# petim0/fly_bProject

Measured on AMD Instinct MI355X. Metric: env-steps/sec (PPO rollout + update), 8192 envs per GPU, higher is better.
Workload: dtype f32 (optimizer step: fp16x2 operand split; rollout policy + critic: bf16x3 operand split; fp32 accumulate)

## Files before the change

### fly_bproject_amd/csrc/fs_common.inc

```
#ifndef FS_IN
#define FS_IN 73
#endif
#ifndef FS_RING
#define FS_RING 4
#endif
typedef short s16x4 __attribute__((ext_vector_type(4)));
constexpr int FS_PX = 96, FS_P1 = 256, FS_P2 = 128, FS_P4 = 32;
template <int PITCH>
__device__ __forceinline__ int fs_key(int r)
{
    if (PITCH % 128 == 0) return ((r & 3) << 2) | ((r >> 2) & 3);
    return (r >> 2) & 3;
}
template <int PITCH>
__device__ __forceinline__ int fs_off(int r, int c) { return r * PITCH + ((((c >> 3) ^ fs_key<PITCH>(r))) << 3) + (c & 7); }
template <int PITCH> constexpr int fs_plane() { return BM * PITCH; }

__device__ __forceinline__ void fs_mfma_v(f32x16& acc, const bf16x8& a, const bf16x8& b)
{
    asm volatile("v_mfma_f32_32x32x16_bf16 %0, %1, %2, %0" : "+v"(acc) : "v"(a), "v"(b));
}
__device__ __forceinline__ void fs_mfma_v0(f32x16& acc, const bf16x8& a, const bf16x8& b)
{
    asm volatile("v_mfma_f32_32x32x16_bf16 %0, %1, %2, 0" : "=&v"(acc) : "v"(a), "v"(b));
}
__device__ __forceinline__ void fs_mfma_vg(f32x16& acc, const bf16x8& a, const bf16x8& b)
{
    asm volatile("s_nop 3\n\tv_mfma_f32_32x32x16_bf16 %0, %1, %2, %0" : "+v"(acc) : "v"(a), "v"(b));
}
__device__ __forceinline__ void fs_mfma_vg0(f32x16& acc, const bf16x8& a, const bf16x8& b)
{
    asm volatile("s_nop 3\n\tv_mfma_f32_32x32x16_bf16 %0, %1, %2, 0" : "=&v"(acc) : "v"(a), "v"(b));
}
__device__ __forceinline__ void fs_mfma_settle(f32x16& acc) { asm volatile("s_nop 7\n\ts_nop 7\n\ts_nop 3" : "+v"(acc)); }
__device__ __forceinline__ void fs_mfma_settle(f32x16& a, f32x16& b) { asm volatile("s_nop 7\n\ts_nop 7\n\ts_nop 3" : "+v"(a), "+v"(b)); }

template <int K, int PITCH, bool SWAP, bool ZERO = true, int HEAD = B3_HEAD>
__device__ __forceinline__ void fs_gemm(const WeightHeadT<HEAD>& head, const u16* __restrict__ Wb, int tile0, const u16* act, int k0,
                                        f32x16& hi, f32x16& lo, int lane)
{
    constexpr int K16 = K / 16;
    constexpr int RING = K16 < FS_RING ? K16 : FS_RING;
    constexpr int ARING = K16 < B3_ARING ? K16 : B3_ARING;
    const int r = lane & 31;
    const int key = fs_key<PITCH>(r);
    const int sh = (k0 >> 3) + (lane >> 5);
    const u16* arow = act + r * PITCH;
    const u16* bp = Wb + (long)tile0 * K16 * 1536 + lane * 8;
    Frag3 b[RING], a[ARING];
    auto aload = [&](Frag3& f, int kb) {
        const u16* q = arow + (((sh + 2 * kb) ^ key) << 3);
#pragma unroll
        for (int p = 0; p < 3; ++p) f.p[p] = *reinterpret_cast<const float4*>(q + p * fs_plane<PITCH>());
    };
#pragma unroll
    for (int s = 0; s < RING; ++s) {
        if (s < ARING) aload(a[s], s);
#pragma unroll
        for (int p = 0; p < 3; ++p)
            b[s].p[p] = s < HEAD ? head.b[s].p[p] : *reinterpret_cast<const float4*>(bp + s * 1536 + p * 512);
    }
#pragma unroll
    for (int kb = 0; kb < K16; ++kb) {
        const int s = kb % RING, sa = kb % ARING;
        __builtin_amdgcn_sched_barrier(0);
        const bf16x8 w0 = as_bf16x8(b[s].p[0]), w1 = as_bf16x8(b[s].p[1]), w2 = as_bf16x8(b[s].p[2]);
        const bf16x8 x0 = as_bf16x8(a[sa].p[0]), x1 = as_bf16x8(a[sa].p[1]), x2 = as_bf16x8(a[sa].p[2]);
        if (ZERO && kb == 0) {
            if (!SWAP) { fs_mfma_v0(lo, w0, x2); fs_mfma_v0(hi, w0, x0); } else { fs_mfma_v0(lo, x2, w0); fs_mfma_v0(hi, x0, w0); }
        } else {
            if (!SWAP) { fs_mfma_v(lo, w0, x2); fs_mfma_v(hi, w0, x0); } else { fs_mfma_v(lo, x2, w0); fs_mfma_v(hi, x0, w0); }
        }
        if (!SWAP) { fs_mfma_v(lo, w2, x0); fs_mfma_v(lo, w1, x1); fs_mfma_v(lo, w0, x1); fs_mfma_v(lo, w1, x0); }
        else { fs_mfma_v(lo, x0, w2); fs_mfma_v(lo, x1, w1); fs_mfma_v(lo, x1, w0); fs_mfma_v(lo, x0, w1); }
        __builtin_amdgcn_sched_barrier(0);
        if (kb + RING < K16) {
#pragma unroll
            for (int p = 0; p < 3; ++p) b[s].p[p] = *reinterpret_cast<const float4*>(bp + (kb + RING) * 1536 + p * 512);
        }
        if (kb + ARING < K16) aload(a[sa], kb + ARING);
    }
    fs_mfma_settle(hi, lo);
    __builtin_amdgcn_sched_barrier(0);
}

template <int K, int PITCH, bool SWAP, bool ZERO, class E, int HOST_GAPS = 6 * (K / 16), int MODE = 0>
struct FsGemmHost {
    static constexpr bool SPLIT = MODE == 1;
    static constexpr int K16 = K / 16, GAPS = 6 * K16, HALF = K16 / 2;
    static constexpr int RING = K16 < FS_RING ? K16 : FS_RING;
    static constexpr int ARING = K16 < B3_ARING ? K16 : B3_ARING;
    static_assert(!SPLIT || K16 == 16, "the split order is written for K = 256");
    static_assert(HOST_GAPS <= GAPS && (MODE == 0 || HOST_GAPS <= 6 * HALF), "the guest must be done when the second half begins");
    static constexpr bool order_ok()
    {
        unsigned seen = 0;
        for (int i = 0; i < K16; ++i) {
            const int kb = kblock(i);
            if (kb < 0 || kb >= K16 || ((seen >> kb) & 1u)) return false;
            if (MODE == 1 && ((kb & 2) != 0) != (i >= HALF)) return false;
            seen |= 1u << kb;
        }
        return true;
    }
    Frag3 b[RING], a[ARING];
    const u16 *arow, *bp;
    int sh, key;
    f32x16 &hi, &lo;
    E& e;
    __device__ __forceinline__ FsGemmHost(f32x16& hi_, f32x16& lo_, E& e_) : hi(hi_), lo(lo_), e(e_) {}
    static constexpr int kblock(int i) { return !SPLIT ? i : (i < HALF ? 4 * (i >> 1) + (i & 1) : 4 * ((i - HALF) >> 1) + 2 + (i & 1)); }
    static_assert(order_ok(), "k-step order");
    __device__ __forceinline__ void aload(Frag3& f, int kb)
    {
        const u16* q = arow + (((sh + 2 * kb) ^ key) << 3);
#pragma unroll
        for (int p = 0; p < 3; ++p) f.p[p] = *reinterpret_cast<const float4*>(q + p * fs_plane<PITCH>());
    }
    __device__ __forceinline__ void bload(Frag3& f, int kb)
    {
#pragma unroll
        for (int p = 0; p < 3; ++p) f.p[p] = *reinterpret_cast<const float4*>(bp + kb * 1536 + p * 512);
    }
    template <int J>
    __device__ __forceinline__ void gap()
    {
        if constexpr (J < HOST_GAPS) {
            constexpr int T0 = J * E::TOTAL / HOST_GAPS, T1 = (J + 1) * E::TOTAL / HOST_GAPS;
            __builtin_amdgcn_sched_barrier(0);
            run<T0, T1>();
            __builtin_amdgcn_sched_barrier(0);
        }
    }
    template <int T, int TE>
    __device__ __forceinline__ void run()
    {
        if constexpr (T < TE) { e.q(T); run<T + 1, TE>(); }
    }
    template <int I>
    __device__ __forceinline__ void steps()
    {
        if constexpr (I < K16) {
            constexpr int s = I % RING, sa = I % ARING;
            if constexpr (MODE != 0 && I == HALF) {
                if (SPLIT) __syncthreads();
#pragma unroll
                for (int u = 0; u < ARING; ++u)
                    if (HALF + u < K16) aload(a[(HALF + u) % ARING], kblock(HALF + u));
            }
            __builtin_amdgcn_sched_barrier(0);
            const bf16x8 w0 = as_bf16x8(b[s].p[0]), w1 = as_bf16x8(b[s].p[1]), w2 = as_bf16x8(b[s].p[2]);
            const bf16x8 x0 = as_bf16x8(a[sa].p[0]), x1 = as_bf16x8(a[sa].p[1]), x2 = as_bf16x8(a[sa].p[2]);
            if constexpr (ZERO && I == 0) {
                if (!SWAP) { fs_mfma_v0(lo, w0, x2); gap<0>(); fs_mfma_v0(hi, w0, x0); } else { fs_mfma_v0(lo, x2, w0); gap<0>(); fs_mfma_v0(hi, x0, w0); }
            } else {
                if (!SWAP) { fs_mfma_v(lo, w0, x2); gap<6 * I>(); fs_mfma_v(hi, w0, x0); } else { fs_mfma_v(lo, x2, w0); gap<6 * I>(); fs_mfma_v(hi, x0, w0); }
            }
            gap<6 * I + 1>();
            if (!SWAP) {
                fs_mfma_v(lo, w2, x0); gap<6 * I + 2>(); fs_mfma_v(lo, w1, x1); gap<6 * I + 3>();
                fs_mfma_v(lo, w0, x1); gap<6 * I + 4>(); fs_mfma_v(lo, w1, x0);
            } else {
                fs_mfma_v(lo, x0, w2); gap<6 * I + 2>(); fs_mfma_v(lo, x1, w1); gap<6 * I + 3>();
                fs_mfma_v(lo, x1, w0); gap<6 * I + 4>(); fs_mfma_v(lo, x0, w1);
            }
            __builtin_amdgcn_sched_barrier(0);
            if constexpr (I + RING < K16) bload(b[s], kblock(I + RING));
            if constexpr (I + ARING < K16 && !(MODE != 0 && I < HALF && I + ARING >= HALF)) aload(a[sa], kblock(I + ARING));
            gap<6 * I + 5>();
            steps<I + 1>();
        }
    }
};
template <int K, int PITCH, bool SWAP, bool ZERO = true, int HEAD = B3_HEAD, int HOST_GAPS = 6 * (K / 16), int MODE = 0, class E>
__device__ __forceinline__ void fs_gemm_host(const WeightHeadT<HEAD>& head, const u16* __restrict__ Wb, int tile0, const u16* act, int k0,
                                             f32x16& hi, f32x16& lo, int lane, E& e)
{
    typedef FsGemmHost<K, PITCH, SWAP, ZERO, E, HOST_GAPS, MODE> G;
    G g(hi, lo, e);
    const int r = lane & 31;
    g.key = fs_key<PITCH>(r);
    g.sh = (k0 >> 3) + (lane >> 5);
    g.arow = act + r * PITCH;
    g.bp = Wb + (long)tile0 * G::K16 * 1536 + lane * 8;
    static_assert(MODE != 1 || HEAD <= 2, "a head is the first k-steps IN ORDER: 0, 1 are the split order's first two as well");
#pragma unroll
    for (int s = 0; s < G::RING; ++s) {
        if (s < G::ARING && (MODE == 0 || s < G::HALF)) g.aload(g.a[s], G::kblock(s));
        if (s < HEAD) {
#pragma unroll
            for (int p = 0; p < 3; ++p) g.b[s].p[p] = head.b[s].p[p];
        } else {
            g.bload(g.b[s], G::kblock(s));
        }
    }
    g.template steps<0>();
    fs_mfma_settle(hi, lo);
    __builtin_amdgcn_sched_barrier(0);
}

template <int T, int TE, class E>
__device__ __forceinline__ void fs_run_ops(E& e)
{
    if constexpr (T < TE) { e.q(T); fs_run_ops<T + 1, TE>(e); }
}
template <int J, int GAPS, class E>
__device__ __forceinline__ void fs_host_gap(E& e)
{
    __builtin_amdgcn_sched_barrier(0);
    fs_run_ops<J * E::TOTAL / GAPS, (J + 1) * E::TOTAL / GAPS>(e);
    __builtin_amdgcn_sched_barrier(0);
}
template <int J0, int GAPS, class E>
__device__ __forceinline__ void fs_dw_host(f32x16& acc, const bf16x8 (&z)[3], const bf16x8 (&a)[3], E& e)
{
    acc = __builtin_amdgcn_mfma_f32_32x32x16_bf16(z[0], a[2], acc, 0, 0, 0); fs_host_gap<J0 + 0, GAPS>(e);
    acc = __builtin_amdgcn_mfma_f32_32x32x16_bf16(z[2], a[0], acc, 0, 0, 0); fs_host_gap<J0 + 1, GAPS>(e);
    acc = __builtin_amdgcn_mfma_f32_32x32x16_bf16(z[1], a[1], acc, 0, 0, 0); fs_host_gap<J0 + 2, GAPS>(e);
    acc = __builtin_amdgcn_mfma_f32_32x32x16_bf16(z[0], a[1], acc, 0, 0, 0); fs_host_gap<J0 + 3, GAPS>(e);
    acc = __builtin_amdgcn_mfma_f32_32x32x16_bf16(z[1], a[0], acc, 0, 0, 0); fs_host_gap<J0 + 4, GAPS>(e);
    acc = __builtin_amdgcn_mfma_f32_32x32x16_bf16(z[0], a[0], acc, 0, 0, 0); fs_host_gap<J0 + 5, GAPS>(e);
}

template <int PITCH>
__device__ __forceinline__ void fs_store4(u16* plane0, int r, int c, const float4& y)
{
    unsigned a0, b0, c0, a1, b1, c1;
    split3x2(y.x, y.y, a0, b0, c0);
    split3x2(y.z, y.w, a1, b1, c1);
    u16* q = plane0 + fs_off<PITCH>(r, c);
    *reinterpret_cast<uint2*>(q) = make_uint2(a0, a1);
    *reinterpret_cast<uint2*>(q + fs_plane<PITCH>()) = make_uint2(b0, b1);
// ... 212 lines not shown
```

### fly_bproject_amd/csrc/mlp_fused_step.inc

```
#include "fs_common.inc"
constexpr int FS_OFF_X = 0;
constexpr int FS_X_HALVES = 3 * BM * FS_PX;
constexpr int FS_OFF_H1 = FS_OFF_X + 2 * FS_X_HALVES;
constexpr int FS_OFF_H2 = FS_OFF_H1 + 3 * BM * FS_P1;
constexpr int FS_OFF_H3 = FS_OFF_H2 + 3 * BM * FS_P2;
constexpr int FS_OFF_R = FS_OFF_H3 + 3 * BM * FS_P2;
constexpr int FS_OFF_Z4 = FS_OFF_R + 4 * BM * MLP_OUT * 2;
constexpr int FS_OFF_F32 = FS_OFF_R + 3 * BM * FS_P2;
constexpr int FS_TAIL_FLOATS = MLP_H1 + MLP_H2 + MLP_H3 + MLP_OUT + 2 * BM + 2 * MLP_OUT + 4;
constexpr int FS_XS_FLOATS = BM * MLP_IN;
constexpr int FS_LDS_BYTES = FS_OFF_F32 * 2 + FS_TAIL_FLOATS * 4;
static_assert(FS_OFF_Z4 + 3 * BM * FS_P4 <= FS_OFF_F32, "split-K partials and the dZ4 planes fit region R side by side");
static_assert(FS_XS_FLOATS * 4 <= 3 * BM * FS_P2 * 2, "the staging block fits H2's region");
static_assert(FS_LDS_BYTES <= 160 * 1024, "fits one CU");

template <int PITCH, bool DUMP>
__device__ __forceinline__ void fs_epilogue_elu(const f32x16& hi, const f32x16& lo, const float* bias, int col0, u16* plane0,
                                                int lane, float* __restrict__ dump_tile, int nvalid)
{
    const int r = lane & 31;
    float4 y[4];
#pragma unroll
    for (int g = 0; g < 4; ++g) {
        const int nb = col0 + acc_n(g, lane);
// ... 491 lines not shown
            f32x16 cs2;
            const bool more = tile + __builtin_amdgcn_readfirstlane(grid_v) < ntiles;
            FsXStoreSlices xc(xs, Xn, tl);
#pragma unroll
            for (int t = 0; t < 2; ++t) {
                const int ct = 2 * wave + t;
                bf16x8 z1f[2][3];
                {
                    f32x16 hi, lo;
                    if (t == 0) fs_gemm<MLP_H2, FS_P2, true>(wt2, PTB + MLP_OFF_PTB2, ct, Z2, 0, hi, lo, lane);
                    else fs_gemm<MLP_H2, FS_P2, true>(wt2b, PTB + MLP_OFF_PTB2, ct, Z2, 0, hi, lo, lane);
                    if (t == 0) { stamp<STAMP>(stamps, 12); if (!STAMP) fs_split(n); }
                    if (STAMP && t == 1) stamp<STAMP>(stamps, 16);
                    if (t == 0 && more) x_fetch(tile + __builtin_amdgcn_readfirstlane(grid_v), tl);
                    bf16x8 hf[2][3], zf[2][3];
#pragma unroll
                    for (int s = 0; s < 2; ++s) fs_trws<FS_P1>(hf[s], H1, tr1, ct, s);
                    fs_trws<FS_P2>(zf[0], Z2, tr2, 0, 0);
                    unsigned q[2][3][4];
                    const fs_u32x4 hw[2][3] = {{__builtin_bit_cast(fs_u32x4, hf[0][0]), __builtin_bit_cast(fs_u32x4, hf[0][1]),
                                                __builtin_bit_cast(fs_u32x4, hf[0][2])},
                                               {__builtin_bit_cast(fs_u32x4, hf[1][0]), __builtin_bit_cast(fs_u32x4, hf[1][1]),
                                                __builtin_bit_cast(fs_u32x4, hf[1][2])}};
                    FsDz1Ops<DUMP> ez(hi, lo, hw, q, DUMP ? dump.dz1 + row0 * MLP_H1 + ct * 1024 : nullptr, lane, nvalid);
#define FS_P8_STEP(C_)                                                                                                            \
                    {                                                                                                             \
                        constexpr int c = (C_), s = c >> 2, nt = c & 3;                                                           \
                        if (c + 1 < 8) fs_trws<FS_P2>(zf[(c + 1) & 1], Z2, tr2, (c + 1) & 3, (c + 1) >> 2);                        \
                        __builtin_amdgcn_sched_barrier(0);                                                                        \
                        fs_dw_host<6 * c, 48>(aW2[nt][t], zf[c & 1], hf[s], ez);                                                  \
                        if (STAMP && t == 0 && c == 3) stamp<STAMP>(stamps, 18);                                                  \
                        if (t == 0 && nt == wave) {                           \
                            if (s == 0) fs_colsum_step<true>(cs2, zf[c & 1]); else fs_colsum_step<false>(cs2, zf[c & 1]);         \
                        }                                                                                                         \
                        __builtin_amdgcn_sched_barrier(0);                                                                        \
                    }
                    FS_P8_STEP(0) FS_P8_STEP(1) FS_P8_STEP(2) FS_P8_STEP(3) FS_P8_STEP(4) FS_P8_STEP(5) FS_P8_STEP(6) FS_P8_STEP(7)
#undef FS_P8_STEP
                    if (STAMP && t == 0) stamp<STAMP>(stamps, 17);
                    bs1[t] += ez.zsum;
#pragma unroll
                    for (int s = 0; s < 2; ++s)
#pragma unroll
                        for (int p = 0; p < 3; ++p) {
                            const fs_u32x4 qq = {q[s][p][0], q[s][p][1], q[s][p][2], q[s][p][3]};
                            z1f[s][p] = __builtin_bit_cast(bf16x8, qq);
                        }
                }
                if (t == 0) {
                    bs2 += fs_colsum_done(cs2);
                    fs_dma_drain();
                    gemm_prefetch_b3<MLP_H2>(wt2b, PTB + MLP_OFF_PTB2, 2 * wave + 1, lane);
                }
                stamp<STAMP>(stamps, t == 0 ? 13 : 15);
                if (!STAMP) fs_split(n);
                {
                    bf16x8 af[2][2][3];
                    fs_trns<FS_PX>(af[0][0], Xc, trx, 0, 0);
                    fs_trns<FS_PX>(af[0][1], Xc, trx, 0, 1);
#pragma unroll
                    for (int kt = 0; kt < 3; ++kt) {
                        if (kt + 1 < 3) {
                            fs_trns<FS_PX>(af[(kt + 1) & 1][0], Xc, trx, kt + 1, 0);
                            fs_trns<FS_PX>(af[(kt + 1) & 1][1], Xc, trx, kt + 1, 1);
                        }
                        __builtin_amdgcn_sched_barrier(0);
                        fs_dw_fill3(aW1[t][kt], z1f[0], af[kt & 1][0], xc, 18 * t + 6 * kt);
                        fs_dw_fill3(aW1[t][kt], z1f[1], af[kt & 1][1], xc, 18 * t + 6 * kt + 3);
                        __builtin_amdgcn_sched_barrier(0);
                    }
                }
                if (t == 0) stamp<STAMP>(stamps, 14);
            }
        }
        stamp<STAMP>(stamps, 10);
        if (!STAMP) fs_split(n);
        __syncthreads();
        stamp<STAMP>(stamps, 11);
        if (!STAMP) fs_split(n);
    }
    if (STAMP) stamps = reinterpret_cast<unsigned long long*>(dump.out) + ((long)blockIdx.x * 64 + 63) * FS_STAMP_SLOTS;
    stamp<STAMP>(stamps, 0);
    if (!STAMP) fs_split(n);

    const int lane = tid & 63;
    const unsigned G = gridDim.x, wg = blockIdx.x;
    constexpr unsigned S1 = fs_pad256(FS_STRIDE1), S2 = fs_pad256(FS_STRIDE2), S3 = fs_pad256(FS_STRIDE3);
    const unsigned o1 = 0, o2 = G * S1, o3 = G * (S1 + S2), o4 = G * (S1 + S2 + S3);
#pragma unroll
    for (int t = 0; t < 2; ++t)
#pragma unroll
        for (int kt = 0; kt < 3; ++kt) fs_store_tile(ws, o1, G, wg, MLP_IN_PAD, 2 * wave + t, kt, aW1[t][kt], lane);
#pragma unroll
    for (int nt = 0; nt < 4; ++nt)
#pragma unroll
        for (int t = 0; t < 2; ++t) fs_store_tile(ws, o2, G, wg, MLP_H1, nt, 2 * wave + t, aW2[nt][t], lane);
#pragma unroll
    for (int a = 0; a < 2; ++a)
#pragma unroll
        for (int b = 0; b < 2; ++b) fs_store_tile(ws, o3, G, wg, MLP_H2, 2 * (wave >> 1) + a, 2 * (wave & 1) + b, aW3[a][b], lane);
    fs_store_tile(ws, o4, G, wg, MLP_H3, 0, wave, aW4, lane);
    if (lane < 32) {
        ws[fs_slab(o2, G, wg, MLP_H2 * MLP_H1 + 32 * wave + lane)] = bs2;
        ws[fs_slab(o3, G, wg, MLP_H3 * MLP_H2 + 32 * wave + lane)] = bs3;
        if (wave == 0) ws[fs_slab(o4, G, wg, MLP_OUT * MLP_H3 + lane)] = bs4;
    }
#pragma unroll
    for (int t = 0; t < 2; ++t) {
        const float v = bs1[t] + __shfl_xor(bs1[t], 32, 64);
        if (lane < 32) ws[fs_slab(o1, G, wg, MLP_H1 * MLP_IN_PAD + 32 * (2 * wave + t) + lane)] = v;
    }
    if (STAMP) {
        asm volatile("s_waitcnt vmcnt(0)" ::: "memory");
        stamp<STAMP>(stamps, 1);
        if (!STAMP) fs_split(n);
        if (threadIdx.x == 0) stamps[2] = realtime_cu();
    }
}

constexpr int FR_OFF_X = 0;
constexpr int FR_OFF_H1 = FR_OFF_X + FS_X_HALVES;
constexpr int FR_OFF_H2 = FR_OFF_H1 + 3 * BM * FS_P1;
constexpr int FR_OFF_H3 = FR_OFF_H2 + 3 * BM * FS_P2;
constexpr int FR_OFF_PART = FR_OFF_H3 + 3 * BM * FS_P2;
constexpr int FR_OFF_F32 = FR_OFF_PART + 4 * BM * MLP_OUT * 2;
constexpr int FR_TAIL_FLOATS = MLP_H1 + MLP_H2 + MLP_H3 + MLP_OUT + 3 * 32 + BM * MLP_NACT + 4;
constexpr int FR_LDS_BYTES = FR_OFF_F32 * 2 + FR_TAIL_FLOATS * 4;
static_assert(BM * MLP_IN * 4 <= 3 * BM * FS_P2 * 2, "the observation block fits H2's region");

struct FrLds {
    u16 *X, *H1, *H2, *H3;
    float *part, *bias1, *bias2, *bias3, *bias4, *sd, *lg, *varcur, *acts, *hld, *obs;
    __device__ __forceinline__ explicit FrLds(u16* lds)
        : X(lds + FR_OFF_X), H1(lds + FR_OFF_H1), H2(lds + FR_OFF_H2), H3(lds + FR_OFF_H3),
          part(reinterpret_cast<float*>(lds + FR_OFF_PART)), bias1(reinterpret_cast<float*>(lds + FR_OFF_F32)), bias2(bias1 + MLP_H1),
          bias3(bias2 + MLP_H2), bias4(bias3 + MLP_H3), sd(bias4 + MLP_OUT), lg(sd + 32), varcur(lg + 32), acts(varcur + 32),
          hld(acts + BM * MLP_NACT), obs(reinterpret_cast<float*>(lds + FR_OFF_H2)) {}
};

__device__ __forceinline__ void policy_tile_fs_setup(const FrLds& L, const float* __restrict__ P)
{
    const int tid = threadIdx.x;
    L.bias1[tid] = P[MLP_OFF_B1 + tid];
    if (tid < MLP_H2) L.bias2[tid] = P[MLP_OFF_B2 + tid];
    else L.bias3[tid - MLP_H2] = P[MLP_OFF_B3 + tid - MLP_H2];
    if (tid < MLP_OUT) L.bias4[tid] = P[MLP_OFF_B4 + tid];
}

__device__ __forceinline__ void policy_tile_fs_head(WeightHeadT<2>& w1, const u16* __restrict__ PB)
{
    const int wave = __builtin_amdgcn_readfirstlane(threadIdx.x >> 6);
    gemm_prefetch_b3<MLP_IN_PAD>(w1, PB + MLP_OFF_PB1, 2 * wave, threadIdx.x & 63);
}
template <bool STAMP = false, bool NORM = false>
__device__ __forceinline__ void policy_tile_fs(const FrLds& L, const long tile, const u16* __restrict__ PB, const float* __restrict__ x,
                                               const long n, float* __restrict__ v_out, const float* __restrict__ smp_eps,
                                               float* __restrict__ smp_act, float* __restrict__ smp_logp, const WeightHeadT<2>& w1,
                                               unsigned long long* stamps = nullptr, const float* norm_tab = nullptr)
{
    const int tid = threadIdx.x, wave = __builtin_amdgcn_readfirstlane(tid >> 6);
    int tl = tid;
    asm volatile("" : "+v"(tl));
    const int lane = tl & 63, r = lane & 31;
    const long row0 = tile * BM;
    const int nvalid = (int)(n - row0 < BM ? n - row0 : BM);
    const int lrow = tl >> 3, lq = tl & 7;
    const bool lin = lrow < nvalid;
    float eps_pre[4];
#pragma unroll
    for (int j = 0; j < 4; ++j)
        eps_pre[j] = (lin && 4 * lq + j < MLP_NACT) ? (smp_eps + row0 * MLP_NACT)[lrow * MLP_NACT + 4 * lq + j] : 0.0f;
    if (x != nullptr) {
        const long total = n * MLP_IN, base = tile * (BM * MLP_IN) + 584L * wave;
        for (int i = lane; i < 584; i += 64) L.obs[584 * wave + i] = base + i < total ? x[base + i] : 0.0f;
    }
    static_assert(BM * MLP_IN == 4 * 584, "eight rows per wave");
    if (tid < 32) {
        const float v = tid < MLP_NACT ? L.varcur[tid] : 1.0f;
        const float s = sqrtf(v);
        L.sd[tid] = s;
        float lg = tid < MLP_NACT ? logf(s) : 0.0f;
        L.lg[tid] = lg;
#pragma unroll
        for (int o = 1; o < 32; o <<= 1) lg += __shfl_xor(lg, o, 32);
        if (tid == 0) L.hld[0] = lg;
    }
    if (NORM) {
        float* row = L.obs + (tl >> 3) * FS_IN;
        const int c0 = 12 * (tl & 7);
#pragma unroll
        for (int j = 0; j < 12; ++j)
            if (c0 + j < FS_IN) row[c0 + j] = obs_norm_apply(row[c0 + j], norm_tab[c0 + j], norm_tab[FS_IN + c0 + j], norm_tab[2 * FS_IN]);
    }
    { FsXStoreSlices xc(L.obs, L.X, tl); xc.all(); }
    __syncthreads();
    stamp<STAMP>(stamps, 1);
    WeightHeadT<2> w4;
    {
        f32x16 hi, lo;
        WeightHeadT<2> w1b, w2a;
        fs_gemm<MLP_IN_PAD, FS_PX, false>(w1, PB + MLP_OFF_PB1, 2 * wave, L.X, 0, hi, lo, lane);
        gemm_prefetch_b3<MLP_IN_PAD>(w1b, PB + MLP_OFF_PB1, 2 * wave + 1, lane);
        fs_epilogue_elu<FS_P1, false>(hi, lo, L.bias1, 64 * wave, L.H1, lane, nullptr, nvalid);
        fs_gemm<MLP_IN_PAD, FS_PX, false>(w1b, PB + MLP_OFF_PB1, 2 * wave + 1, L.X, 0, hi, lo, lane);
        gemm_prefetch_b3<MLP_H2>(w2a, PB + MLP_OFF_PB2, wave, lane);
        fs_epilogue_elu<FS_P1, false>(hi, lo, L.bias1, 64 * wave + 32, L.H1, lane, nullptr, nvalid);
        __syncthreads();
        stamp<STAMP>(stamps, 2);
        WeightHeadT<2> w2b, w3;
        gemm_prefetch_b3<MLP_H2>(w2b, PB + MLP_OFF_PB2 + 3 * MLP_H2 * (MLP_H1 / 2), wave, lane);
        fs_gemm<MLP_H2, FS_P1, false>(w2a, PB + MLP_OFF_PB2, wave, L.H1, 0, hi, lo, lane);
        fs_gemm<MLP_H2, FS_P1, false, false>(w2b, PB + MLP_OFF_PB2 + 3 * MLP_H2 * (MLP_H1 / 2), wave, L.H1, MLP_H1 / 2, hi, lo, lane);
        gemm_prefetch_b3<MLP_H2>(w3, PB + MLP_OFF_PB3, wave, lane);
        fs_epilogue_elu<FS_P2, false>(hi, lo, L.bias2, 32 * wave, L.H2, lane, nullptr, nvalid);
        __syncthreads();
        stamp<STAMP>(stamps, 3);
        gemm_prefetch_b3<32>(w4, PB + MLP_OFF_PB4 + (long)(2 * wave) * 1536, 0, lane);
        fs_gemm<MLP_H2, FS_P2, false>(w3, PB + MLP_OFF_PB3, wave, L.H2, 0, hi, lo, lane);
        fs_epilogue_elu<FS_P2, false>(hi, lo, L.bias3, 32 * wave, L.H3, lane, nullptr, nvalid);
        __syncthreads();
        stamp<STAMP>(stamps, 4);
    }
    {
        f32x16 hi, lo;
        fs_gemm<32, FS_P2, false>(w4, PB + MLP_OFF_PB4 + (long)(2 * wave) * 1536, 0, L.H3, 32 * wave, hi, lo, lane);
        float* pw = L.part + wave * (BM * MLP_OUT);
#pragma unroll
        for (int g = 0; g < 4; ++g)
            *reinterpret_cast<float4*>(pw + r * MLP_OUT + 4 * ((acc_n(g, lane) >> 2) ^ ((r >> 1) & 7))) =
                make_float4(hi[4 * g] + lo[4 * g], hi[4 * g + 1] + lo[4 * g + 1], hi[4 * g + 2] + lo[4 * g + 2],
                            hi[4 * g + 3] + lo[4 * g + 3]);
    }
    __syncthreads();
    stamp<STAMP>(stamps, 5);
    {
        const int c0 = 4 * lq;
        const int cs = 4 * (lq ^ ((lrow >> 1) & 7));
        const float4 p0 = *reinterpret_cast<const float4*>(L.part + lrow * MLP_OUT + cs);
        const float4 p1 = *reinterpret_cast<const float4*>(L.part + BM * MLP_OUT + lrow * MLP_OUT + cs);
        const float4 p2 = *reinterpret_cast<const float4*>(L.part + 2 * BM * MLP_OUT + lrow * MLP_OUT + cs);
        const float4 p3 = *reinterpret_cast<const float4*>(L.part + 3 * BM * MLP_OUT + lrow * MLP_OUT + cs);
        const float4 b4 = *reinterpret_cast<const float4*>(L.bias4 + c0);
        const float4 s4 = *reinterpret_cast<const float4*>(L.sd + c0);
        const float hld = L.hld[0];
        const float zz[4] = {(((p0.x + p1.x) + p2.x) + p3.x) + b4.x, (((p0.y + p1.y) + p2.y) + p3.y) + b4.y,
                             (((p0.z + p1.z) + p2.z) + p3.z) + b4.z, (((p0.w + p1.w) + p2.w) + p3.w) + b4.w};
        const float sdv[4] = {s4.x, s4.y, s4.z, s4.w};
        float a[4], xsq[4], yv[4];
#pragma unroll
        for (int j = 0; j < 4; ++j) {
            const int col = c0 + j;
            const float y = (col < MLP_NACT) ? elu(zz[j]) : ((col == MLP_NACT) ? zz[j] : 0.0f);
            yv[j] = y;
            a[j] = 0.0f; xsq[j] = 0.0f;
            if (col < MLP_NACT && lin) {
                a[j] = y + sdv[j] * eps_pre[j];
                const float xj = (a[j] - y) / sdv[j];
                xsq[j] = xj * xj;
            }
        }
        const float M = fs_sum8((xsq[0] + xsq[1]) + (xsq[2] + xsq[3]));
        if (lin) {
            if (v_out && lq == MLP_NACT / 4) (v_out + row0)[lrow] = yv[MLP_NACT % 4];
#pragma unroll
            for (int j = 0; j < 4; ++j)
                if (c0 + j < MLP_NACT) {
                    const float ac = fminf(fmaxf(a[j], -1.0f), 1.0f);
                    (smp_act + row0 * MLP_NACT)[lrow * MLP_NACT + c0 + j] = ac;
                    L.acts[lrow * MLP_NACT + c0 + j] = ac;
                }
            if (lq == 0) (smp_logp + row0)[lrow] = gauss_logp(M, hld);
        }
    }
    __syncthreads();
}
```

### fly_bproject_amd/csrc/mlp_mfma.hip

```cpp
#include <hip/hip_runtime.h>
#include <stdint.h>
#include <type_traits>
#include <cstdio>
#include <cstdlib>
#include "flyhip.h"
#include "mlp_layout.h"
#include "obs_norm.h"
#include "domain_rand.h"
#include "launch.h"

namespace {

#include "loss_head.inc"
#include "mlp_gemm.inc"
#include "fs_stamp.inc"
#include "mlp_forward.inc"
#include "mlp_backward.inc"
#include "mlp_grad_w.inc"
#include "mlp_fused_step.inc"
#include "mlp_adam.inc"
#include "fly_body.inc"

constexpr int RS_LDS_FLOATS = FWD_LDS_FLOATS > ENVS_PER_BLOCK * FLY_NUM_OBS ? FWD_LDS_FLOATS : ENVS_PER_BLOCK * FLY_NUM_OBS;
constexpr int RS_B3_LDS_FLOATS = FWD_B3_LDS_FLOATS > ENVS_PER_BLOCK * FLY_NUM_OBS ? FWD_B3_LDS_FLOATS : ENVS_PER_BLOCK * FLY_NUM_OBS;
static_assert(ENVS_PER_BLOCK == BM && BLOCK == THREADS, "one forward tile = one env block");
constexpr int NORM_LDS_FLOATS = OBS_NORM_TABLE + 1;
static_assert(MLP_IN == OBS_NORM_COLS && OBS_NORM_TABLE <= THREADS, "one table entry per thread");

template <bool B3, bool NORM = false, bool DR = false>
__global__ __launch_bounds__(THREADS, B3 ? 1 : 2) void rollout_step_kernel(
    const FlyConfig* __restrict__ c, FlyBuffers b, const float* __restrict__ P, const void* __restrict__ PF,
    const float* __restrict__ x, long n, const float* __restrict__ eps, const float* __restrict__ var, int var_steps,
    float var_decay, float var_min, float* __restrict__ act, float* __restrict__ logp, float* __restrict__ v_out,
    const int* __restrict__ var_base)
{
    constexpr int ARENA = B3 ? RS_B3_LDS_FLOATS : RS_LDS_FLOATS;
    __shared__ __attribute__((aligned(16))) float lds[ARENA + (NORM ? NORM_LDS_FLOATS : 0)];
    float* const norm_tab = NORM ? lds + ARENA : nullptr;
    if (NORM) obs_norm_load(norm_tab, c);
    var_steps -= var_base ? *var_base : 0;
    constexpr int PH_ALL = PH_SCALE | PH_RESET | PH_INTEGRATE | PH_OBS | PH_PROGRESS | PH_REWARD;
    FlyRegs st;
    fly_load<PH_ALL, DR>(st, c, b, blockIdx.x);
    if (NORM) __syncthreads();
    if (B3)
        forward_body_b3<false, false, NORM>(lds, blockIdx.x, 1L << 40, P, static_cast<const u16*>(PF), x, n, nullptr, v_out, nullptr,
                                            nullptr, nullptr, nullptr, eps, var, act, logp, nullptr, var_steps, var_decay, var_min,
                                            nullptr, nullptr, false, norm_tab);
    else
        forward_body<false, false, NORM>(lds, blockIdx.x, 1L << 40, P, static_cast<const float*>(PF), x, n, nullptr, v_out, nullptr,
                                         nullptr, nullptr, nullptr, eps, var, act, logp, nullptr, var_steps, var_decay, var_min,
                                         norm_tab);
    __builtin_amdgcn_fence(__ATOMIC_RELEASE, "workgroup");
    __builtin_amdgcn_s_waitcnt(0);
    __syncthreads();
    fly_body<PH_ALL, DR>(c, act, b, lds, blockIdx.x, st);
}

__device__ __forceinline__ void store_pose(float* __restrict__ poses, int t, const FlyRegs& nx)
{
    const int sub = threadIdx.x;
    if (sub >= LANES_PER_ENV) return;
    float* p = poses + (long)t * FLY_POSE_FLOATS;
    if (sub < FLY_NUM_LEGS) {
#pragma unroll
        for (int i = 0; i < 3; ++i) p[7 + 3 * sub + i] = nx.jq[i];
    }
    if (sub == LANES_PER_ENV - 1) {
        p[0] = nx.r.px; p[1] = nx.r.py; p[2] = nx.r.pz; p[3] = nx.r.qx; p[4] = nx.r.qy; p[5] = nx.r.qz; p[6] = nx.r.qw;
    }
}

template <bool B3, int WPS, bool REC, bool NORM = false, bool DR = false>
__global__ __launch_bounds__(THREADS, WPS) void rollout_all_kernel(
    const FlyConfig* __restrict__ c, FlyBuffers b, const float* __restrict__ P, const void* __restrict__ PF,
    float* __restrict__ obs_ring, long n, const float* __restrict__ eps_all, const float* __restrict__ var, float var_decay,
    float var_min, float* __restrict__ act_all, float* __restrict__ logp_all, float* __restrict__ v_ring,
    float* __restrict__ reward_all, int T, const int* __restrict__ rows_applied, int64_t* __restrict__ reset_rows,
    int64_t* __restrict__ progress_rows, float* __restrict__ poses)
{
    constexpr int ARENA = B3 ? RS_B3_LDS_FLOATS : RS_LDS_FLOATS;
    __shared__ __attribute__((aligned(16))) float lds[ARENA + 32 + BM * MLP_NACT + (NORM ? NORM_LDS_FLOATS : 0)];
    float* const norm_tab = NORM ? lds + ARENA + 32 + BM * MLP_NACT : nullptr;
    if (NORM) obs_norm_load(norm_tab, c);
    constexpr int PH_ALL = PH_SCALE | PH_RESET | PH_INTEGRATE | PH_OBS | PH_PROGRESS | PH_REWARD;
    float* varcur = lds + ARENA;
    float* acts = B3 ? lds + ARENA + 32 : nullptr;
    if (threadIdx.x < MLP_NACT) varcur[threadIdx.x] = var[threadIdx.x];
    FlyRegs st;
    fly_load<PH_ALL, DR>(st, c, b, blockIdx.x);
    __syncthreads();
    const bool whole = (long)(blockIdx.x + 1) * BM <= n;
    for (int t = 0; t < T; ++t) {
        const float* x = obs_ring + (long)t * n * FLY_NUM_OBS;
        float* act = act_all + (long)t * n * MLP_NACT;
        b.obs = obs_ring + (long)(t + 1) * n * FLY_NUM_OBS;
        b.reward = reward_all + (long)t * n;
        if (reset_rows) { b.reset = reset_rows + (long)t * n; b.progress = progress_rows + (long)t * n; }
        const bool in_lds = B3 && whole;
        if (B3)
            forward_body_b3<false, false, NORM>(lds, blockIdx.x, 1L << 40, P, static_cast<const u16*>(PF), x, n, nullptr,
                                                v_ring + (long)t * n, nullptr, nullptr, nullptr, nullptr, eps_all + (long)t * n * MLP_NACT,
                                                varcur, act, logp_all + (long)t * n, nullptr, 0, var_decay, var_min,
                                                in_lds && t > 0 ? lds : nullptr, in_lds ? acts : nullptr, t > 0, norm_tab);
        else
            forward_body<false, false, NORM>(lds, blockIdx.x, 1L << 40, P, static_cast<const float*>(PF), x, n, nullptr,
                                             v_ring + (long)t * n, nullptr, nullptr, nullptr, nullptr, eps_all + (long)t * n * MLP_NACT,
                                             varcur, act, logp_all + (long)t * n, nullptr, 0, var_decay, var_min, norm_tab);
        if (!in_lds) {
            __builtin_amdgcn_fence(__ATOMIC_RELEASE, "workgroup");
            __builtin_amdgcn_s_waitcnt(0);
        }
        __syncthreads();
        FlyRegs nx;
        fly_body<PH_ALL, DR>(c, act, b, lds, blockIdx.x, st, &nx, in_lds ? acts : nullptr);
        if (REC && blockIdx.x == 0) store_pose(poses, t, nx);
        st = nx;
        if (threadIdx.x < MLP_NACT && var_decay > 0.0f) varcur[threadIdx.x] = fmaxf(var_min, varcur[threadIdx.x] - var_decay);
        if (!in_lds) asm volatile("s_waitcnt vmcnt(0)" ::: "memory");
        __syncthreads();
    }
}

template <bool STAMP, bool MULTI, bool REC, bool NORM = false, bool DR = false>
__global__ __launch_bounds__(THREADS, 1) void rollout_all_fs_kernel(
    const FlyConfig* __restrict__ c, FlyBuffers b, const float* __restrict__ P, const u16* __restrict__ PB,
    float* __restrict__ obs_ring, long n, const float* __restrict__ eps_all, const float* __restrict__ var, float var_decay,
    float var_min, float* __restrict__ act_all, float* __restrict__ logp_all, float* __restrict__ v_ring,
    float* __restrict__ reward_all, int T, int64_t* __restrict__ reset_rows, int64_t* __restrict__ progress_rows,
    void* __restrict__ aux)
{
    static_assert(!(STAMP && REC) && !(STAMP && NORM) && !(STAMP && DR), "the stamped diagnostic form neither records, normalises nor randomises");
    unsigned long long* const stamps = static_cast<unsigned long long*>(aux);
    float* const poses = static_cast<float*>(aux);
    extern __shared__ __attribute__((aligned(16))) u16 fr_lds[];
    const FrLds L(fr_lds);
    constexpr int PH_ALL = PH_SCALE | PH_RESET | PH_INTEGRATE | PH_OBS | PH_PROGRESS | PH_REWARD;
    policy_tile_fs_setup(L, P);
    float* const norm_tab = NORM ? reinterpret_cast<float*>(fr_lds) + FR_LDS_BYTES / 4 : nullptr;
    if (NORM) obs_norm_load(norm_tab, c);
    int64_t* const reset0 = b.reset;
    int64_t* const progress0 = b.progress;
    const long ntiles = n / BM;
    long tile = blockIdx.x;
    do {
        unsigned long long* st_tile = STAMP ? stamps + tile * (T + 1) * 8 : nullptr;
        if (threadIdx.x < 32) L.varcur[threadIdx.x] = threadIdx.x < MLP_NACT ? var[threadIdx.x] : 1.0f;
        b.reset = reset0; b.progress = progress0;
        FlyRegs st;
        fly_load<PH_ALL, DR>(st, c, b, (int)tile);
        WeightHeadT<2> w1;
        policy_tile_fs_head(w1, PB);
        __syncthreads();
        if (STAMP && threadIdx.x == 0) st_tile[6] = realtime_cu();
        for (int t = 0; t < T; ++t) {
            stamp<STAMP>(st_tile, 8 * t);
            float* act = act_all + (long)t * n * MLP_NACT;
            b.obs = obs_ring + (long)(t + 1) * n * FLY_NUM_OBS;
            b.reward = reward_all + (long)t * n;
            if (reset_rows) { b.reset = reset_rows + (long)t * n; b.progress = progress_rows + (long)t * n; }
            policy_tile_fs<STAMP, NORM>(L, tile, PB, t == 0 ? obs_ring : nullptr, n, v_ring + (long)t * n, eps_all + (long)t * n * MLP_NACT,
                                        act, logp_all + (long)t * n, w1, STAMP ? st_tile + 8 * t : nullptr, norm_tab);
            stamp<STAMP>(st_tile, 8 * t + 7);
            policy_tile_fs_head(w1, PB);
            FlyRegs nx;
            fly_body<PH_ALL, DR>(c, act, b, L.obs, (int)tile, st, &nx, L.acts);
            if (REC && tile == 0) store_pose(poses, t, nx);
            st = nx;
            if (threadIdx.x < MLP_NACT && var_decay > 0.0f) L.varcur[threadIdx.x] = fmaxf(var_min, L.varcur[threadIdx.x] - var_decay);
            __syncthreads();
        }
        stamp<STAMP>(st_tile, 8 * T);
        if (STAMP && threadIdx.x == 0) st_tile[8 * T + 1] = realtime_cu();
        tile += gridDim.x;
    } while (MULTI && tile < ntiles);
}

}

extern "C" hipError_t flyhip_launch_rollout_all(const FlyConfig* dcfg, const FlyBuffers* b, const float* P, const float* PF,
                                                float* obs_ring, int64_t n, const float* eps_all, const float* var,
                                                float var_decay, float var_min, float* act_all, float* logp_all, float* v_ring,
                                                float* reward_all, int T, const int* rows_applied, const uint16_t* PB,
                                                int64_t* reset_rows, int64_t* progress_rows, void* stream,
                                                unsigned long long* stamps, float* poses, int norm, int dr)
{
    const dim3 grid((unsigned)((n + BM - 1) / BM));
    const int cus = device_cus();
    const bool one_per_cu = (int)grid.x <= cus;
    const char* fs_env = getenv("FLY_ROLLOUT_FS");
    const bool fs_off = fs_env != nullptr && fs_env[0] == '0';
    if (stamps && (poses || norm || dr)) return hipErrorInvalidValue;
    const bool rec = poses != nullptr;
    if (PB && n % BM == 0 && !fs_off) {
        const dim3 grid_fs(one_per_cu ? grid.x : (unsigned)cus);
        static_assert(FR_LDS_BYTES % 4 == 0, "the table follows the image");
        auto fs = [&](void* aux, auto S, auto M, auto R, auto N, auto D) {
            return launch_kernel<rollout_all_fs_kernel<S.value, M.value, R.value, N.value, D.value>>(
                grid_fs, THREADS, FR_LDS_BYTES + (N.value ? NORM_LDS_FLOATS * 4 : 0), stream, dcfg, *b, P, PB, obs_ring, (long)n, eps_all,
                var, var_decay, var_min, act_all, logp_all, v_ring, reward_all, T, reset_rows, progress_rows, aux);
        };
        constexpr std::false_type no{};
        const bool multi = !one_per_cu;
        if (stamps) return with_bools([&](auto M) { return fs(stamps, std::true_type{}, M, no, no, no); }, multi);
        return with_bools([&](auto M, auto R, auto N, auto D) { return fs(poses, no, M, R, N, D); }, multi, rec, norm != 0, dr != 0);
    }
    if (stamps) return hipErrorInvalidValue;
    auto ra = [&](auto B3, auto WPS, const void* pf) {
        return with_bools([&](auto R, auto N, auto D) {
            return launch_kernel<rollout_all_kernel<B3.value, WPS.value, R.value, N.value, D.value>>(
                grid, THREADS, 0, stream, dcfg, *b, P, pf, obs_ring, (long)n, eps_all, var, var_decay, var_min, act_all, logp_all, v_ring,
                reward_all, T, rows_applied, reset_rows, progress_rows, poses);
        }, rec, norm != 0, dr != 0);
    };
    if (PB) return ra(std::true_type{}, int_c<1>{}, PB);
    return one_per_cu ? ra(std::false_type{}, int_c<1>{}, PF) : ra(std::false_type{}, int_c<2>{}, PF);
}

extern "C" hipError_t flyhip_launch_mlp_forward(const float* P, const float* PF, const float* x, int64_t n, float* mu_out,
                                                float* v_out, float* out_save, float* h1_save, float* h2_save,
                                                float* h3_save, const uint16_t* PB, void* stream)
{
    if (PB) {
        const long tiles = (n + BM - 1) / BM;
        const int grid = (int)tiles;
        hipLaunchKernelGGL(mlp_forward_b3_kernel, dim3(grid), dim3(THREADS), 0, (hipStream_t)stream, P, PB, x, (long)n, mu_out,
                           v_out, out_save, h1_save, h2_save, h3_save, (const float*)nullptr, (const float*)nullptr,
                           (float*)nullptr, (float*)nullptr, 0, 0.0f, 0.0f, (const int*)nullptr);
        return hipGetLastError();
    }
    const long tiles = (n + BM - 1) / BM;
    const int grid = (int)(tiles <= 4 * PERSIST_GRID ? tiles : PERSIST_GRID);
    hipLaunchKernelGGL(mlp_forward_kernel<false>, dim3(grid), dim3(THREADS), 0, (hipStream_t)stream, P, PF, x, (long)n,
                       mu_out, v_out, out_save, h1_save, h2_save, h3_save, (const float*)nullptr, (const float*)nullptr,
                       (float*)nullptr, (float*)nullptr, (unsigned long long*)nullptr, 0, 0.0f, 0.0f, (const int*)nullptr);
    return hipGetLastError();
}

extern "C" hipError_t flyhip_launch_mlp_forward_sample(const float* P, const float* PF, const float* x, int64_t n,
                                                       const float* eps, const float* var, int var_steps,
                                                       float var_decay, float var_min, float* act_out,
                                                       float* logp_out, float* mu_out, float* v_out, const uint16_t* PB,
                                                       const int* var_base, void* stream)
{
    if (PB) {
        const long tiles = (n + BM - 1) / BM;
        const int grid = (int)tiles;
        hipLaunchKernelGGL(mlp_forward_b3_kernel, dim3(grid), dim3(THREADS), 0, (hipStream_t)stream, P, PB, x, (long)n, mu_out,
                           v_out, (float*)nullptr, (float*)nullptr, (float*)nullptr, (float*)nullptr, eps, var, act_out,
                           logp_out, var_steps, var_decay, var_min, var_base);
        return hipGetLastError();
    }
    const long tiles = (n + BM - 1) / BM;
    const int grid = (int)(tiles <= 4 * PERSIST_GRID ? tiles : PERSIST_GRID);
    hipLaunchKernelGGL(mlp_forward_kernel<false>, dim3(grid), dim3(THREADS), 0, (hipStream_t)stream, P, PF, x, (long)n,
                       mu_out, v_out, (float*)nullptr, (float*)nullptr, (float*)nullptr, (float*)nullptr, eps,
                       var, act_out, logp_out, (unsigned long long*)nullptr, var_steps, var_decay, var_min, var_base);
    return hipGetLastError();
}

extern "C" int flyhip_debug_mlp_forward_stamped(const float* P, const float* PF, const float* x, int64_t n,
                                                float* out_save, float* h1_save, float* h2_save, float* h3_save,
                                                unsigned long long* stamps, void* stream, int grid_override)
{
    const long tiles = (n + BM - 1) / BM;
    const int grid = grid_override > 0 ? grid_override : (int)(tiles <= 4 * PERSIST_GRID ? tiles : PERSIST_GRID);
    hipLaunchKernelGGL(mlp_forward_kernel<true>, dim3(grid), dim3(THREADS), 0, (hipStream_t)stream, P, PF, x, (long)n,
                       (float*)nullptr, (float*)nullptr, out_save, h1_save, h2_save, h3_save, (const float*)nullptr,
                       (const float*)nullptr, (float*)nullptr, (float*)nullptr, stamps, 0, 0.0f, 0.0f, (const int*)nullptr);
    return (int)hipGetLastError();
}

extern "C" hipError_t flyhip_launch_mlp_backward_dx(const float* PT, const float* out_saved, const float* h1,
                                                    const float* h2, const float* h3, const float* action,
                                                    const float* old_logp, const float* adv, const float* target,
                                                    const float* var, int64_t n, float inv_batch, float clip,
                                                    float* dz4, float* dz3, float* dz2, float* dz1, float* loss_part,
                                                    const uint16_t* PTB, void* stream)
{
    if (PTB) {
        hipLaunchKernelGGL(mlp_backward_dx_b3_kernel, dim3((unsigned)((n + BM - 1) / BM)), dim3(THREADS), 0, (hipStream_t)stream,
                           PTB, out_saved, h1, h2, h3, action, old_logp, adv, target, var, (long)n, inv_batch, clip, dz4, dz3,
                           dz2, dz1, loss_part);
        return hipGetLastError();
    }
    const int grid = (int)((n + BM - 1) / BM);
    hipLaunchKernelGGL(mlp_backward_dx_kernel, dim3(grid), dim3(THREADS), 0, (hipStream_t)stream, PT, out_saved,
                       h1, h2, h3, action, old_logp, adv, target, var, (long)n, inv_batch, clip, dz4, dz3, dz2, dz1,
                       loss_part);
    return hipGetLastError();
}

static int kGradWgs[4] = {80, 100, 52, 24};
static int kGradWgsB3[4] = {72, 88, 64, 32};
static bool gw_env_read = false;
static void gw_read_env()
{
    if (gw_env_read) return;
    gw_env_read = true;
    const char* e = getenv("FLYHIP_GW_SPLIT");
    int v[4];
    if (e && sscanf(e, "%d,%d,%d,%d", &v[0], &v[1], &v[2], &v[3]) == 4 && v[0] > 0 && v[1] > 0 && v[2] > 0 && v[3] > 0 &&
        v[0] + v[1] + v[2] + v[3] <= 1024)
        for (int i = 0; i < 4; ++i) kGradWgs[i] = kGradWgsB3[i] = v[i];
}

static int g_fb_consumer_shift = 0;
extern "C" void flyhip_debug_set_fwd_bwd_consumer_shift(int shift) { g_fb_consumer_shift = shift; }

extern "C" hipError_t flyhip_launch_mlp_fwd_bwd(const float* P, const float* PF, const float* PT, const float* x, int64_t n,
                                                float* out_save, float* h1_save, float* h2_save, float* h3_save,
                                                const float* action, const float* old_logp, const float* adv,
                                                const float* target, const float* var, float inv_batch, float clip,
                                                float* dz4, float* dz3, float* dz2, float* dz1, float* loss_part,
                                                int* flags, int epoch, int* err, const uint16_t* PB, const uint16_t* PTB,
// ... 169 lines not shown
```

Before: 70.57 million.

## Keep layer-2 and output-head policy weights resident in AGPRs across rollout steps

Layer-2 and output-layer weight fragments are loaded once per kernel into accumulation registers (AGPRs) and reused on every timestep and tile. A new GEMM variant feeds MFMA directly from those registers instead of streaming weights from global memory through a prefetch ring. This removes repeated weight loads from the rollout loop. In exchange it holds a large block of AGPRs for the whole kernel, which can cut occupancy or cause spills.

Measured after the change: 70.91 million, median of 6. About the same (+0.5%).

```diff
diff --git a/fly_bproject_amd/csrc/fs_common.inc b/fly_bproject_amd/csrc/fs_common.inc
--- a/fly_bproject_amd/csrc/fs_common.inc
+++ b/fly_bproject_amd/csrc/fs_common.inc
@@ -78,6 +78,58 @@
 #pragma unroll
             for (int p = 0; p < 3; ++p) b[s].p[p] = *reinterpret_cast<const float4*>(bp + (kb + RING) * 1536 + p * 512);
         }
+        if (kb + ARING < K16) aload(a[sa], kb + ARING);
+    }
+    fs_mfma_settle(hi, lo);
+    __builtin_amdgcn_sched_barrier(0);
+}
+
+struct FragA { bf16x8 p[3]; };
+__device__ __forceinline__ void fs_hold(FragA& f)
+{
+#pragma unroll
+    for (int p = 0; p < 3; ++p) asm volatile("" : "+a"(f.p[p]));
+}
+__device__ __forceinline__ void fs_load_resident(FragA& f, const u16* bp)
+{
+#pragma unroll
+    for (int p = 0; p < 3; ++p) f.p[p] = as_bf16x8(*reinterpret_cast<const float4*>(bp + p * 512));
+    fs_hold(f);
+}
+__device__ __forceinline__ void fs_mfma_a(f32x16& acc, const bf16x8& w, const bf16x8& x)
+{
+    asm volatile("v_mfma_f32_32x32x16_bf16 %0, %1, %2, %0" : "+v"(acc) : "a"(w), "v"(x));
+}
+__device__ __forceinline__ void fs_mfma_a0(f32x16& acc, const bf16x8& w, const bf16x8& x)
+{
+    asm volatile("v_mfma_f32_32x32x16_bf16 %0, %1, %2, 0" : "=&v"(acc) : "a"(w), "v"(x));
+}
+template <int K, int PITCH, bool ZERO = true>
+__device__ __forceinline__ void fs_gemm_resident(const FragA (&w)[K / 16], const u16* act, int k0, f32x16& hi, f32x16& lo, int lane)
+{
+    constexpr int K16 = K / 16;
+    constexpr int ARING = K16 < B3_ARING ? K16 : B3_ARING;
+    const int r = lane & 31;
+    const int key = fs_key<PITCH>(r);
+    const int sh = (k0 >> 3) + (lane >> 5);
+    const u16* arow = act + r * PITCH;
+    Frag3 a[ARING];
+    auto aload = [&](Frag3& f, int kb) {
+        const u16* q = arow + (((sh + 2 * kb) ^ key) << 3);
+#pragma unroll
+        for (int p = 0; p < 3; ++p) f.p[p] = *reinterpret_cast<const float4*>(q + p * fs_plane<PITCH>());
+    };
+#pragma unroll
+    for (int s = 0; s < ARING; ++s) aload(a[s], s);
+#pragma unroll
+    for (int kb = 0; kb < K16; ++kb) {
+        const int sa = kb % ARING;
+        __builtin_amdgcn_sched_barrier(0);
+        const bf16x8 x0 = as_bf16x8(a[sa].p[0]), x1 = as_bf16x8(a[sa].p[1]), x2 = as_bf16x8(a[sa].p[2]);
+        if (ZERO && kb == 0) { fs_mfma_a0(lo, w[kb].p[0], x2); fs_mfma_a0(hi, w[kb].p[0], x0); }
+        else { fs_mfma_a(lo, w[kb].p[0], x2); fs_mfma_a(hi, w[kb].p[0], x0); }
+        fs_mfma_a(lo, w[kb].p[2], x0); fs_mfma_a(lo, w[kb].p[1], x1); fs_mfma_a(lo, w[kb].p[0], x1); fs_mfma_a(lo, w[kb].p[1], x0);
+        __builtin_amdgcn_sched_barrier(0);
         if (kb + ARING < K16) aload(a[sa], kb + ARING);
     }
     fs_mfma_settle(hi, lo);
diff --git a/fly_bproject_amd/csrc/mlp_fused_step.inc b/fly_bproject_amd/csrc/mlp_fused_step.inc
--- a/fly_bproject_amd/csrc/mlp_fused_step.inc
+++ b/fly_bproject_amd/csrc/mlp_fused_step.inc
@@ -667,11 +667,24 @@
     const int wave = __builtin_amdgcn_readfirstlane(threadIdx.x >> 6);
     gemm_prefetch_b3<MLP_IN_PAD>(w1, PB + MLP_OFF_PB1, 2 * wave, threadIdx.x & 63);
 }
+struct PolicyResident { FragA w2[2][MLP_H2 / 16], w4[2]; };
+__device__ __forceinline__ void policy_tile_fs_resident(PolicyResident& w, const u16* __restrict__ PB)
+{
+    const int wave = __builtin_amdgcn_readfirstlane(threadIdx.x >> 6), lane = threadIdx.x & 63;
+#pragma unroll
+    for (int h = 0; h < 2; ++h)
+#pragma unroll
+        for (int kb = 0; kb < MLP_H2 / 16; ++kb)
+            fs_load_resident(w.w2[h][kb], PB + MLP_OFF_PB2 + h * (3 * MLP_H2 * (MLP_H1 / 2)) + ((long)wave * (MLP_H2 / 16) + kb) * 1536 + lane * 8);
+#pragma unroll
+    for (int kb = 0; kb < 2; ++kb) fs_load_resident(w.w4[kb], PB + MLP_OFF_PB4 + (long)(2 * wave + kb) * 1536 + lane * 8);
+}
 template <bool STAMP = false, bool NORM = false>
 __device__ __forceinline__ void policy_tile_fs(const FrLds& L, const long tile, const u16* __restrict__ PB, const float* __restrict__ x,
                                                const long n, float* __restrict__ v_out, const float* __restrict__ smp_eps,
                                                float* __restrict__ smp_act, float* __restrict__ smp_logp, const WeightHeadT<2>& w1,
-                                               unsigned long long* stamps = nullptr, const float* norm_tab = nullptr)
+                                               const PolicyResident& wr, unsigned long long* stamps = nullptr,
+                                               const float* norm_tab = nullptr)
 {
     const int tid = threadIdx.x, wave = __builtin_amdgcn_readfirstlane(tid >> 6);
     int tl = tid;
@@ -710,27 +723,23 @@
     { FsXStoreSlices xc(L.obs, L.X, tl); xc.all(); }
     __syncthreads();
     stamp<STAMP>(stamps, 1);
-    WeightHeadT<2> w4;
     {
         f32x16 hi, lo;
-        WeightHeadT<2> w1b, w2a;
+        WeightHeadT<2> w1b;
         fs_gemm<MLP_IN_PAD, FS_PX, false>(w1, PB + MLP_OFF_PB1, 2 * wave, L.X, 0, hi, lo, lane);
         gemm_prefetch_b3<MLP_IN_PAD>(w1b, PB + MLP_OFF_PB1, 2 * wave + 1, lane);
         fs_epilogue_elu<FS_P1, false>(hi, lo, L.bias1, 64 * wave, L.H1, lane, nullptr, nvalid);
         fs_gemm<MLP_IN_PAD, FS_PX, false>(w1b, PB + MLP_OFF_PB1, 2 * wave + 1, L.X, 0, hi, lo, lane);
-        gemm_prefetch_b3<MLP_H2>(w2a, PB + MLP_OFF_PB2, wave, lane);
         fs_epilogue_elu<FS_P1, false>(hi, lo, L.bias1, 64 * wave + 32, L.H1, lane, nullptr, nvalid);
         __syncthreads();
         stamp<STAMP>(stamps, 2);
-        WeightHeadT<2> w2b, w3;
-        gemm_prefetch_b3<MLP_H2>(w2b, PB + MLP_OFF_PB2 + 3 * MLP_H2 * (MLP_H1 / 2), wave, lane);
-        fs_gemm<MLP_H2, FS_P1, false>(w2a, PB + MLP_OFF_PB2, wave, L.H1, 0, hi, lo, lane);
-        fs_gemm<MLP_H2, FS_P1, false, false>(w2b, PB + MLP_OFF_PB2 + 3 * MLP_H2 * (MLP_H1 / 2), wave, L.H1, MLP_H1 / 2, hi, lo, lane);
+        WeightHeadT<2> w3;
+        fs_gemm_resident<MLP_H2, FS_P1>(wr.w2[0], L.H1, 0, hi, lo, lane);
+        fs_gemm_resident<MLP_H2, FS_P1, false>(wr.w2[1], L.H1, MLP_H1 / 2, hi, lo, lane);
         gemm_prefetch_b3<MLP_H2>(w3, PB + MLP_OFF_PB3, wave, lane);
         fs_epilogue_elu<FS_P2, false>(hi, lo, L.bias2, 32 * wave, L.H2, lane, nullptr, nvalid);
         __syncthreads();
         stamp<STAMP>(stamps, 3);
-        gemm_prefetch_b3<32>(w4, PB + MLP_OFF_PB4 + (long)(2 * wave) * 1536, 0, lane);
         fs_gemm<MLP_H2, FS_P2, false>(w3, PB + MLP_OFF_PB3, wave, L.H2, 0, hi, lo, lane);
         fs_epilogue_elu<FS_P2, false>(hi, lo, L.bias3, 32 * wave, L.H3, lane, nullptr, nvalid);
         __syncthreads();
@@ -738,7 +747,7 @@
     }
     {
         f32x16 hi, lo;
-        fs_gemm<32, FS_P2, false>(w4, PB + MLP_OFF_PB4 + (long)(2 * wave) * 1536, 0, L.H3, 32 * wave, hi, lo, lane);
+        fs_gemm_resident<32, FS_P2>(wr.w4, L.H3, 32 * wave, hi, lo, lane);
         float* pw = L.part + wave * (BM * MLP_OUT);
 #pragma unroll
         for (int g = 0; g < 4; ++g)
diff --git a/fly_bproject_amd/csrc/mlp_mfma.hip b/fly_bproject_amd/csrc/mlp_mfma.hip
--- a/fly_bproject_amd/csrc/mlp_mfma.hip
+++ b/fly_bproject_amd/csrc/mlp_mfma.hip
@@ -143,6 +143,8 @@
     int64_t* const progress0 = b.progress;
     const long ntiles = n / BM;
     long tile = blockIdx.x;
+    PolicyResident wr;
+    policy_tile_fs_resident(wr, PB);
     do {
         unsigned long long* st_tile = STAMP ? stamps + tile * (T + 1) * 8 : nullptr;
         if (threadIdx.x < 32) L.varcur[threadIdx.x] = threadIdx.x < MLP_NACT ? var[threadIdx.x] : 1.0f;
@@ -160,7 +162,7 @@
             b.reward = reward_all + (long)t * n;
             if (reset_rows) { b.reset = reset_rows + (long)t * n; b.progress = progress_rows + (long)t * n; }
             policy_tile_fs<STAMP, NORM>(L, tile, PB, t == 0 ? obs_ring : nullptr, n, v_ring + (long)t * n, eps_all + (long)t * n * MLP_NACT,
-                                        act, logp_all + (long)t * n, w1, STAMP ? st_tile + 8 * t : nullptr, norm_tab);
+                                        act, logp_all + (long)t * n, w1, wr, STAMP ? st_tile + 8 * t : nullptr, norm_tab);
             stamp<STAMP>(st_tile, 8 * t + 7);
             policy_tile_fs_head(w1, PB);
             FlyRegs nx;
```
